# mizeller/OnePose_ST

Hardware: AMD Instinct MI355X
Metric: query frames/sec (2D-3D match+PnP) @ 7k x 4800 d256; 1/2/4/8 GPU (higher is better)
Workload: dtype bf16x3 (split-bf16 MFMA, f32 accumulate)

## Files before the change

### onepose_st_amd/csrc/prep.hip

```cpp
#include "tile.h"

namespace {

__global__ __launch_bounds__(256) void pe_add_transpose_kernel(const float* __restrict__ feat, const float* __restrict__ pe,
                                                               float* __restrict__ out, int Cc, int M) {
    __shared__ float tile[32][33];
    const int tx = threadIdx.x & 31, ty = threadIdx.x >> 5;
    const int m0 = blockIdx.x * 32, c0 = blockIdx.y * 32, b = blockIdx.z;
    const float* f = feat + (size_t)b * Cc * M;
#pragma unroll
    for (int k = 0; k < 4; ++k) {
        const int c = c0 + ty + 8 * k, m = m0 + tx;
        tile[ty + 8 * k][tx] = (c < Cc && m < M) ? f[(size_t)c * M + m] : 0.f;
    }
    __syncthreads();
    float* o = out + (size_t)b * M * Cc;
#pragma unroll
    for (int k = 0; k < 4; ++k) {
        const int m = m0 + ty + 8 * k, c = c0 + tx;
        if (m < M && c < Cc) o[(size_t)m * Cc + c] = tile[tx][ty + 8 * k] + (pe ? pe[(size_t)m * Cc + c] : 0.f);
    }
}

constexpr int KS_THREADS = 1024, KS_WAVES = KS_THREADS / 64;

__global__ __launch_bounds__(KS_THREADS) void kpt_stats_kernel(const float* __restrict__ kpts, long long bs, float* __restrict__ stats, int B, int N) {
    __shared__ float red[KS_WAVES][9];
    const int b = blockIdx.x, tid = threadIdx.x, lane = tid & 63, wave = tid >> 6;
    const float* k = kpts + (size_t)b * bs;
    float s[3] = {0.f, 0.f, 0.f}, mn[3] = {INFINITY, INFINITY, INFINITY}, mx[3] = {-INFINITY, -INFINITY, -INFINITY};
#pragma unroll 4
    for (int i = tid; i < N; i += KS_THREADS) {
#pragma unroll
        for (int d = 0; d < 3; ++d) {
            const float v = k[(size_t)i * 3 + d];
            s[d] += v; mn[d] = fminf(mn[d], v); mx[d] = fmaxf(mx[d], v);
        }
    }
#pragma unroll
    for (int d = 0; d < 3; ++d) {
        s[d] = wave_sum(s[d]);
        mx[d] = wave_max(mx[d]);
        mn[d] = -wave_max(-mn[d]);
    }
    if (lane == 0) {
#pragma unroll
        for (int d = 0; d < 3; ++d) { red[wave][d] = s[d]; red[wave][3 + d] = mn[d]; red[wave][6 + d] = mx[d]; }
    }
    __syncthreads();
    if (tid == 0) {
        float ext = 0.f;
        for (int d = 0; d < 3; ++d) {
            float sum = 0.f, lo = INFINITY, hi = -INFINITY;
            for (int w = 0; w < KS_WAVES; ++w) {
                sum += red[w][d];
                lo = fminf(lo, red[w][3 + d]);
                hi = fmaxf(hi, red[w][6 + d]);
            }
            stats[4 * b + d] = sum / (float)N;
            ext = fmaxf(ext, hi - lo);
        }
        stats[4 * b + 3] = 0.f;
        if (b == 0) stats[4 * B] = ext * 0.6f;
    }
}

constexpr int KD = 256;
constexpr int L0 = 8 + OPHIP_PAD, L1 = 32 + OPHIP_PAD, L2 = 64 + OPHIP_PAD, L3 = 128 + OPHIP_PAD, LO = KD + OPHIP_PAD;

struct KptArgs {
    const float* kpts; long long kbs;
    const float* stats;
    const float* desc; long long dbs;
    const f32x4 *w1, *w2, *w3, *w4;
    const float *b1, *b2, *b3, *b4;
    float* out;
    int B, N;
};

__global__ __launch_bounds__(256) void kpt_encode_kernel(KptArgs p) {
    extern __shared__ __attribute__((aligned(16))) float smem[];
    float* A0 = smem;
    float* A1 = A0 + 32 * L0;
    float* A2 = A1 + 32 * L1;
    float* A3 = A2 + 32 * L2;
    float* Ot = A3 + 32 * L3;
    const int tid = threadIdx.x, lane = tid & 63, wave = tid >> 6;
    const int r = lane & 31, h = lane >> 5;
    const int n0 = blockIdx.x * 32, b = blockIdx.y;
    const float scaling = p.stats[4 * p.B];
    if (tid < 32 * 8) {
        const int row = tid >> 3, d = tid & 7;
        float v = 0.f;
        if (d < 3 && n0 + row < p.N) v = (p.kpts[(size_t)b * p.kbs + (size_t)(n0 + row) * 3 + d] - p.stats[4 * b + d]) / scaling;
        A0[row * L0 + d] = v;
    }
    const float* dsc = p.desc + (size_t)b * p.dbs;
    {
        float dv[KD * 32 / 256];
        const int n = tid & 31, cb = tid >> 5;
        const bool live = n0 + n < p.N;
#pragma unroll
        for (int k = 0; k < KD * 32 / 256; ++k) dv[k] = live ? dsc[(size_t)(cb + 8 * k) * p.N + n0 + n] : 0.f;
#pragma unroll
        for (int k = 0; k < KD * 32 / 256; ++k) Ot[n * LO + cb + 8 * k] = dv[k];
    }
    __syncthreads();
    if (wave == 0) {
        f32x16 acc[1] = {zero16()};
        gemm_lds_x_packed<1, 1>(acc, A0 + r * L0 + 4 * h, 1, p.w1 + lane, 64);
        const float bias = p.b1[r];
#pragma unroll
        for (int reg = 0; reg < 16; ++reg) acc[0][reg] += bias;
        acc_to_lds(acc[0], A1, L1, 0, lane);
    }
    __syncthreads();
    rows_layernorm<32, false, true>(A1, L1, nullptr, nullptr, 1e-5f, wave, lane);
    __syncthreads();
    if (wave < 2) {
        f32x16 acc[1] = {zero16()};
        gemm_lds_x_packed<1>(acc, A1 + r * L1 + 4 * h, 4, p.w2 + (size_t)wave * 4 * 64 + lane, 4 * 64);
        const float bias = p.b2[32 * wave + r];
#pragma unroll
        for (int reg = 0; reg < 16; ++reg) acc[0][reg] += bias;
        acc_to_lds(acc[0], A2, L2, 32 * wave, lane);
    }
    __syncthreads();
    rows_layernorm<64, false, true>(A2, L2, nullptr, nullptr, 1e-5f, wave, lane);
    __syncthreads();
    {
        f32x16 acc[1] = {zero16()};
        gemm_lds_x_packed<1>(acc, A2 + r * L2 + 4 * h, 8, p.w3 + (size_t)wave * 8 * 64 + lane, 8 * 64);
        const float bias = p.b3[32 * wave + r];
#pragma unroll
        for (int reg = 0; reg < 16; ++reg) acc[0][reg] += bias;
        acc_to_lds(acc[0], A3, L3, 32 * wave, lane);
    }
    __syncthreads();
    rows_layernorm<128, false, true>(A3, L3, nullptr, nullptr, 1e-5f, wave, lane);
    __syncthreads();
    {
        f32x16 acc[2] = {zero16(), zero16()};
        gemm_lds_x_packed<2>(acc, A3 + r * L3 + 4 * h, 16, p.w4 + (size_t)(2 * wave) * 16 * 64 + lane, 16 * 64);
#pragma unroll
        for (int t = 0; t < 2; ++t) {
            const int c = 64 * wave + 32 * t + r;
            const float bias = p.b4[c];
#pragma unroll
            for (int reg = 0; reg < 16; ++reg) {
                const int row = acc_row(reg, h);
                Ot[row * LO + c] = Ot[row * LO + c] + (acc[t][reg] + bias);
            }
        }
    }
    __syncthreads();
    float* o = p.out + (size_t)b * p.N * KD;
    for (int rr = 0; rr < 8; ++rr) {
        const int row = 8 * wave + rr;
        if (n0 + row < p.N)
            *reinterpret_cast<f32x4*>(o + (size_t)(n0 + row) * KD + 4 * lane) = *reinterpret_cast<const f32x4*>(Ot + row * LO + 4 * lane);
    }
}

__global__ __launch_bounds__(256) void transpose_cl_kernel(const float* __restrict__ in, float* __restrict__ out, int Cc, int L) {
    __shared__ float tile[32][33];
    const int tx = threadIdx.x & 31, ty = threadIdx.x >> 5;
    const int l0 = blockIdx.x * 32, c0 = blockIdx.y * 32, b = blockIdx.z;
#pragma unroll
    for (int k = 0; k < 4; ++k) {
        const int c = c0 + ty + 8 * k, l = l0 + tx;
        tile[ty + 8 * k][tx] = (c < Cc && l < L) ? in[((size_t)b * Cc + c) * L + l] : 0.f;
    }
    __syncthreads();
#pragma unroll
    for (int k = 0; k < 4; ++k) {
        const int l = l0 + ty + 8 * k, c = c0 + tx;
        if (l < L && c < Cc) out[((size_t)b * L + l) * Cc + c] = tile[tx][ty + 8 * k];
    }
}

__global__ __launch_bounds__(256) void transpose_c128_kernel(const float* __restrict__ in, float* __restrict__ out, int L) {
    __shared__ float tile[128][33];
    const int tid = threadIdx.x, l0 = blockIdx.x * 32, b = blockIdx.y;
    const float* src = in + (size_t)b * 128 * L;
    const int lx = tid & 31, cy = tid >> 5;
#pragma unroll
    for (int k = 0; k < 16; ++k) {
        const int c = cy + 8 * k;
        tile[c][lx] = (l0 + lx < L) ? src[(size_t)c * L + l0 + lx] : 0.f;
    }
    __syncthreads();
    float* dst = out + (size_t)b * L * 128;
    const int p = tid >> 3, q0 = tid & 7;
    if (l0 + p < L) {
#pragma unroll
        for (int m = 0; m < 4; ++m) {
            const int q = q0 + 8 * m;
            f32x4 v = {tile[4 * q][p], tile[4 * q + 1][p], tile[4 * q + 2][p], tile[4 * q + 3][p]};
            *reinterpret_cast<f32x4*>(dst + (size_t)(l0 + p) * 128 + 4 * q) = v;
        }
    }
}

__global__ __launch_bounds__(256) void crop_resize_kernel(const unsigned char* __restrict__ img, int H, int W, int x0, int y0, int wb, int hb,
                                                          int S, float* __restrict__ out) {
    const int X = blockIdx.x * 32 + (threadIdx.x & 31), Y = blockIdx.y * 8 + (threadIdx.x >> 5);
    if (X >= S || Y >= S) return;
    const float inv = (float)wb / (float)S;
    const float u = ((float)X - 0.5f * (float)S) * inv + 0.5f * (float)wb;
    const float v = ((float)Y - 0.5f * (float)S) * inv + 0.5f * (float)hb;
    const float fu = floorf(u), fv = floorf(v);
    const int i0 = (int)fu, j0 = (int)fv;
    const float a = u - fu, b = v - fv;
    auto px = [&](int i, int j) -> float {
        if (i < 0 || i >= wb || j < 0 || j >= hb) return 0.f;
        const int x = x0 + i, y = y0 + j;
        return (x >= 0 && x < W && y >= 0 && y < H) ? (float)img[(size_t)y * W + x] : 0.f;
    };
    const float val = (1.f - b) * ((1.f - a) * px(i0, j0) + a * px(i0 + 1, j0)) + b * ((1.f - a) * px(i0, j0 + 1) + a * px(i0 + 1, j0 + 1));
    out[(size_t)Y * S + X] = fminf(fmaxf(rintf(val), 0.f), 255.f) / 255.0f;
}

}

extern "C" int ophip_crop_resize_gray(const unsigned char* image, int H, int W, int x0, int y0, int x1, int y1, int S, float* out, void* stream) {
    if (!image || !out) return ophip_bad_arg(__func__, "null pointer");
    if (H < 1 || W < 1 || S < 1 || x1 <= x0 || y1 <= y0) return ophip_bad_arg(__func__, "bad sizes (need x1 > x0, y1 > y0)");
    OPHIP_LAUNCH("crop_resize", (hipStream_t)stream, crop_resize_kernel, dim3((S + 31) / 32, (S + 7) / 8), dim3(256), 0, (hipStream_t)stream,
                 image, H, W, x0, y0, x1 - x0, y1 - y0, S, out);
    OPHIP_CHECK_LAUNCH();
    return 0;
}

extern "C" int ophip_pe_add_transpose(const float* feat_nchw, const float* pe_nlc, float* out_nlc, int B, int C, int M, void* stream) {
    if (!feat_nchw || !out_nlc) return ophip_bad_arg(__func__, "null pointer");
    if (B < 1 || C < 1 || M < 1) return ophip_bad_arg(__func__, "bad sizes");
    OPHIP_LAUNCH("pe_add_transpose", (hipStream_t)stream, pe_add_transpose_kernel, dim3((M + 31) / 32, (C + 31) / 32, B), dim3(256), 0, (hipStream_t)stream,
                       feat_nchw, pe_nlc, out_nlc, C, M);
    OPHIP_CHECK_LAUNCH();
    return 0;
}

extern "C" int ophip_transpose_cl(const float* in_bcl, float* out_blc, int B, int C, int L, void* stream) {
    if (!in_bcl || !out_blc) return ophip_bad_arg(__func__, "null pointer");
    if (C == 128) {
        OPHIP_LAUNCH("transpose_cl", (hipStream_t)stream, transpose_c128_kernel, dim3((L + 31) / 32, B), dim3(256), 0, (hipStream_t)stream, in_bcl, out_blc, L);
        OPHIP_CHECK_LAUNCH();
        return 0;
    }
    OPHIP_LAUNCH("transpose_cl", (hipStream_t)stream, transpose_cl_kernel, dim3((L + 31) / 32, (C + 31) / 32, B), dim3(256), 0, (hipStream_t)stream, in_bcl, out_blc, C, L);
    OPHIP_CHECK_LAUNCH();
    return 0;
}

extern "C" int ophip_kpt_encode(const float* keypoints3d, long long kpts_bstride, const float* desc_bcn, long long desc_bstride,
                                const float* wpack, float* stats, float* out_bnc, int B, int N, void* stream_) {
    if (!keypoints3d || !desc_bcn || !wpack || !stats || !out_bnc) return ophip_bad_arg(__func__, "null pointer");
    if (B < 1 || N < 1) return ophip_bad_arg(__func__, "bad sizes");
    hipStream_t stream = (hipStream_t)stream_;
    OPHIP_LAUNCH("kpt_stats", stream, kpt_stats_kernel, dim3(B), dim3(KS_THREADS), 0, stream, keypoints3d, kpts_bstride, stats, B, N);
    OPHIP_CHECK_LAUNCH();
    KptArgs a;
    a.kpts = keypoints3d; a.kbs = kpts_bstride; a.stats = stats; a.desc = desc_bcn; a.dbs = desc_bstride;
    const float* w = wpack;
    a.w1 = reinterpret_cast<const f32x4*>(w); w += 32 * 8;
    a.w2 = reinterpret_cast<const f32x4*>(w); w += 64 * 32;
    a.w3 = reinterpret_cast<const f32x4*>(w); w += 128 * 64;
    a.w4 = reinterpret_cast<const f32x4*>(w); w += 256 * 128;
    a.b1 = w; a.b2 = w + 32; a.b3 = w + 96; a.b4 = w + 224;
    a.out = out_bnc; a.B = B; a.N = N;
    const size_t lds = (size_t)(32 * (L0 + L1 + L2 + L3 + LO)) * sizeof(float);
    if (int rc = ophip_lds_attr(reinterpret_cast<const void*>(kpt_encode_kernel), lds, "hipFuncSetAttribute(kpt_encode)")) return rc;
    OPHIP_LAUNCH("kpt_encode", stream, kpt_encode_kernel, dim3((N + 31) / 32, B), dim3(256), lds, stream, a);
    OPHIP_CHECK_LAUNCH();
    return 0;
}
```

Baseline: 1546.

## Fuse keypoint stats into encoder, vectorize transposes, preload MLP weights into registers

Removes the separate kpt_stats launch: every encoder block now recomputes the keypoint mean and extent itself (redundant per-block reduction over N points) before normalizing. The MLP weights are preloaded into registers, with a ring prefetch for the last layer, and the layernorm+ReLU uses DPP/permlane reductions. The descriptor loads are vectorized. The transpose and pe-add kernels are rewritten to use f32x4 loads and stores with a rotated LDS tile. This cuts one launch and several memory passes, but adds redundant reduction work in each block and more register pressure.

```diff
diff --git a/onepose_st_amd/csrc/prep.hip b/onepose_st_amd/csrc/prep.hip
--- a/onepose_st_amd/csrc/prep.hip
+++ b/onepose_st_amd/csrc/prep.hip
@@ -2,8 +2,72 @@
 
 namespace {
 
+constexpr int TR_C = 128;
+constexpr int TR_T_FINE = 64;
+constexpr int TR_T_PE = 32;
+
+template <int T, bool VEC, bool PE>
+__device__ __forceinline__ void transpose_tile(const float* __restrict__ src, const float* __restrict__ pe, float* __restrict__ dst,
+                                               int C, int L, int l0, int c0, f32x4* tile) {
+    constexpr int LQ = T / 4, CQ = 256 / LQ, PASS = 32 / CQ, ROT = 16 / LQ, ROWS = T / 8;
+    static_assert(T == 32 || T == 64, "tile of 32 or 64 positions");
+    const int tid = threadIdx.x;
+    const int lq = tid % LQ, cq = tid / LQ, l = l0 + 4 * lq;
+    f32x4 v[PASS][4];
+#pragma unroll
+    for (int p = 0; p < PASS; ++p)
+#pragma unroll
+        for (int i = 0; i < 4; ++i) {
+            const float* s = src + (size_t)(c0 + 4 * (cq + CQ * p) + i) * L;
+            if (VEC) {
+                v[p][i] = *reinterpret_cast<const f32x4*>(s + (l < L ? l : 0));
+            } else {
+#pragma unroll
+                for (int j = 0; j < 4; ++j) v[p][i][j] = s[l + j < L ? l + j : 0];
+            }
+        }
+    const int q = tid & 31, r8 = tid >> 5;
+    f32x4 o[ROWS];
+#pragma unroll
+    for (int k = 0; k < ROWS; ++k) o[k] = f32x4{0.f, 0.f, 0.f, 0.f};
+    if (PE && pe) {
+#pragma unroll
+        for (int k = 0; k < ROWS; ++k) {
+            const int lr = l0 + r8 + 8 * k;
+            o[k] = *reinterpret_cast<const f32x4*>(pe + (size_t)(lr < L ? lr : 0) * C + c0 + 4 * q);
+        }
+    }
+#pragma unroll
+    for (int p = 0; p < PASS; ++p)
+#pragma unroll
+        for (int j = 0; j < 4; ++j) {
+            const f32x4 t = {v[p][0][j], v[p][1][j], v[p][2][j], v[p][3][j]};
+            tile[(4 * lq + j) * 32 + ((cq + CQ * p + ROT * lq) & 31)] = t;
+        }
+    __syncthreads();
+#pragma unroll
+    for (int k = 0; k < ROWS; ++k) {
+        const int row = r8 + 8 * k;
+        const f32x4 t = tile[row * 32 + ((q + ROT * (row >> 2)) & 31)];
+        o[k] = PE ? t + o[k] : t;
+    }
+#pragma unroll
+    for (int k = 0; k < ROWS; ++k) {
+        const int lr = l0 + r8 + 8 * k;
+        if (lr < L) *reinterpret_cast<f32x4*>(dst + (size_t)lr * C + c0 + 4 * q) = o[k];
+    }
+}
+
+template <bool VEC>
 __global__ __launch_bounds__(256) void pe_add_transpose_kernel(const float* __restrict__ feat, const float* __restrict__ pe,
                                                                float* __restrict__ out, int Cc, int M) {
+    __shared__ f32x4 tile[TR_T_PE * 32];
+    const int b = blockIdx.z;
+    transpose_tile<TR_T_PE, VEC, true>(feat + (size_t)b * Cc * M, pe, out + (size_t)b * M * Cc, Cc, M, blockIdx.x * TR_T_PE, blockIdx.y * TR_C, tile);
+}
+
+__global__ __launch_bounds__(256) void pe_add_transpose_generic_kernel(const float* __restrict__ feat, const float* __restrict__ pe,
+                                                                       float* __restrict__ out, int Cc, int M) {
     __shared__ float tile[32][33];
     const int tx = threadIdx.x & 31, ty = threadIdx.x >> 5;
     const int m0 = blockIdx.x * 32, c0 = blockIdx.y * 32, b = blockIdx.z;
@@ -23,62 +87,157 @@
 }
 
 constexpr int KS_THREADS = 1024, KS_WAVES = KS_THREADS / 64;
-
-__global__ __launch_bounds__(KS_THREADS) void kpt_stats_kernel(const float* __restrict__ kpts, long long bs, float* __restrict__ stats, int B, int N) {
-    __shared__ float red[KS_WAVES][9];
-    const int b = blockIdx.x, tid = threadIdx.x, lane = tid & 63, wave = tid >> 6;
-    const float* k = kpts + (size_t)b * bs;
-    float s[3] = {0.f, 0.f, 0.f}, mn[3] = {INFINITY, INFINITY, INFINITY}, mx[3] = {-INFINITY, -INFINITY, -INFINITY};
-#pragma unroll 4
-    for (int i = tid; i < N; i += KS_THREADS) {
-#pragma unroll
-        for (int d = 0; d < 3; ++d) {
-            const float v = k[(size_t)i * 3 + d];
-            s[d] += v; mn[d] = fminf(mn[d], v); mx[d] = fmaxf(mx[d], v);
-        }
-    }
-#pragma unroll
-    for (int d = 0; d < 3; ++d) {
-        s[d] = wave_sum(s[d]);
-        mx[d] = wave_max(mx[d]);
-        mn[d] = -wave_max(-mn[d]);
-    }
-    if (lane == 0) {
-#pragma unroll
-        for (int d = 0; d < 3; ++d) { red[wave][d] = s[d]; red[wave][3 + d] = mn[d]; red[wave][6 + d] = mx[d]; }
-    }
-    __syncthreads();
-    if (tid == 0) {
-        float ext = 0.f;
-        for (int d = 0; d < 3; ++d) {
-            float sum = 0.f, lo = INFINITY, hi = -INFINITY;
-            for (int w = 0; w < KS_WAVES; ++w) {
-                sum += red[w][d];
-                lo = fminf(lo, red[w][3 + d]);
-                hi = fmaxf(hi, red[w][6 + d]);
-            }
-            stats[4 * b + d] = sum / (float)N;
-            ext = fmaxf(ext, hi - lo);
-        }
-        stats[4 * b + 3] = 0.f;
-        if (b == 0) stats[4 * B] = ext * 0.6f;
-    }
-}
-
 constexpr int KD = 256;
 constexpr int L0 = 8 + OPHIP_PAD, L1 = 32 + OPHIP_PAD, L2 = 64 + OPHIP_PAD, L3 = 128 + OPHIP_PAD, LO = KD + OPHIP_PAD;
 
 struct KptArgs {
     const float* kpts; long long kbs;
-    const float* stats;
+    float* stats;
     const float* desc; long long dbs;
     const f32x4 *w1, *w2, *w3, *w4;
     const float *b1, *b2, *b3, *b4;
     float* out;
     int B, N;
+    int dvec;
 };
 
-__global__ __launch_bounds__(256) void kpt_encode_kernel(KptArgs p) {
+__device__ __forceinline__ float lane_xor4(float v) {
+    const int u = __builtin_bit_cast(int, v);
+    int t = __builtin_amdgcn_update_dpp(u, u, 0x104, 0xf, 0x5, false);
+    t = __builtin_amdgcn_update_dpp(t, u, 0x114, 0xf, 0xa, false);
+    return __builtin_bit_cast(float, t);
+}
+__device__ __forceinline__ float wave_sum_from16(float v) {
+    const unsigned u = __builtin_bit_cast(unsigned, v);
+    auto a = __builtin_amdgcn_permlane16_swap(u, u, false, false);
+    const unsigned a0 = a[0], a1 = a[1];
+    v = __builtin_bit_cast(float, a0) + __builtin_bit_cast(float, a1);
+    v += dpp_f<0x128>(v);
+    v += lane_xor4(v);
+    v += dpp_f<0x4E>(v);
+    v += dpp_f<0xB1>(v);
+    return v;
+}
+__device__ __forceinline__ float wave_sum_valu(float v) { return wave_sum_from16(swap32_sum(v)); }
+
+__device__ __forceinline__ void kpt_partials(const float* __restrict__ k, int N, float (*red)[9], int wave, int lane) {
+    float s[4][3], mn[4][3], mx[4][3];
+#pragma unroll
+    for (int v = 0; v < 4; ++v)
+#pragma unroll
+        for (int d = 0; d < 3; ++d) { s[v][d] = 0.f; mn[v][d] = INFINITY; mx[v][d] = -INFINITY; }
+#pragma unroll 2
+    for (int i0 = 64 * wave + lane; i0 < N; i0 += KS_THREADS) {
+#pragma unroll
+        for (int v = 0; v < 4; ++v) {
+            const int i = i0 + 256 * v;
+            const bool in = i < N;
+            const float* kp = k + (size_t)(in ? i : 0) * 3;
+#pragma unroll
+            for (int d = 0; d < 3; ++d) {
+                const float x = kp[d];
+                s[v][d] = in ? s[v][d] + x : s[v][d];
+                mn[v][d] = in ? fminf(mn[v][d], x) : mn[v][d];
+                mx[v][d] = in ? fmaxf(mx[v][d], x) : mx[v][d];
+            }
+        }
+    }
+    float lo[4][3], hi[4][3];
+#pragma unroll
+    for (int v = 0; v < 4; ++v)
+#pragma unroll
+        for (int d = 0; d < 3; ++d) {
+            s[v][d] = wave_sum_valu(s[v][d]);
+            hi[v][d] = wave_max_dpp(mx[v][d]);
+            lo[v][d] = -wave_max_dpp(-mn[v][d]);
+        }
+    if (lane == 0) {
+#pragma unroll
+        for (int v = 0; v < 4; ++v)
+#pragma unroll
+            for (int d = 0; d < 3; ++d) { red[wave + 4 * v][d] = s[v][d]; red[wave + 4 * v][3 + d] = lo[v][d]; red[wave + 4 * v][6 + d] = hi[v][d]; }
+    }
+}
+
+template <int KB>
+__device__ __forceinline__ void gemm_lds_x_regs(f32x16& acc, const float* lds_a, const f32x4 (&w)[KB]) {
+#pragma unroll
+    for (int kb = 0; kb < KB; ++kb) acc = mfma4(*reinterpret_cast<const f32x4*>(lds_a + 8 * kb), w[kb], acc);
+}
+
+template <int NT, int PD>
+__device__ __forceinline__ void ring_fill(f32x4 (&ring)[PD][NT], const f32x4* __restrict__ wfrag, int tstride) {
+#pragma unroll
+    for (int p = 0; p < PD; ++p)
+#pragma unroll
+        for (int t = 0; t < NT; ++t) ring[p][t] = wfrag[(size_t)t * tstride + (size_t)p * 64];
+}
+template <int NT, int PD>
+__device__ __forceinline__ void gemm_lds_x_ring(f32x16 (&acc)[NT], const float* lds_a, int kblocks, const f32x4* __restrict__ wfrag, int tstride,
+                                                f32x4 (&ring)[PD][NT]) {
+    for (int kb0 = 0; kb0 < kblocks; kb0 += PD) {
+#pragma unroll
+        for (int p = 0; p < PD; ++p) {
+            const int kb = kb0 + p;
+            const f32x4 a = *reinterpret_cast<const f32x4*>(lds_a + 8 * kb);
+#pragma unroll
+            for (int t = 0; t < NT; ++t) acc[t] = mfma4(a, ring[p][t], acc[t]);
+            const int kn = (kb + PD < kblocks) ? kb + PD : kblocks - 1;
+#pragma unroll
+            for (int t = 0; t < NT; ++t) ring[p][t] = wfrag[(size_t)t * tstride + (size_t)kn * 64];
+            __builtin_amdgcn_sched_barrier(0);
+        }
+    }
+}
+
+template <int C>
+__device__ __forceinline__ float norm_rstd(float qsum, float eps) { return 1.0f / sqrtf(qsum * (1.0f / C) + eps); }
+
+template <int C>
+__device__ __forceinline__ void rows_norm_relu8(float* img, int ld, float eps, int wave, int lane) {
+#pragma clang fp contract(off)
+    constexpr int PER = (C + 63) / 64;
+    static_assert(C % 64 == 0 ? PER <= 2 : PER == 1, "one or two whole elements per lane, or part of a wave");
+    float d[8][PER], s[8], q[8];
+#pragma unroll
+    for (int rr = 0; rr < 8; ++rr) {
+        const float* row = img + (8 * wave + rr) * ld;
+        s[rr] = 0.f;
+#pragma unroll
+        for (int e = 0; e < PER; ++e) {
+            const int c = lane + 64 * e;
+            d[rr][e] = (c < C) ? row[c] : 0.f;
+            s[rr] += d[rr][e];
+        }
+    }
+#pragma unroll
+    for (int rr = 0; rr < 8; ++rr) {
+        const float sum = wave_sum_valu(s[rr]);
+#pragma unroll
+        for (int e = 0; e < PER; ++e) d[rr][e] = __builtin_fmaf(sum, -(1.0f / C), d[rr][e]);
+        const float d0 = (lane < C) ? d[rr][0] : 0.f;
+        if (PER == 1) {
+            q[rr] = wave_sum_from16(__builtin_fmaf(d0, d0, __shfl_xor(d0 * d0, 32, 64)));
+        } else {
+            q[rr] = wave_sum_valu(__builtin_fmaf(d0, d0, d[rr][PER - 1] * d[rr][PER - 1]));
+        }
+    }
+#pragma unroll
+    for (int rr = 0; rr < 8; ++rr) {
+        float* row = img + (8 * wave + rr) * ld;
+        const float rstd = norm_rstd<C>(q[rr], eps);
+#pragma unroll
+        for (int e = 0; e < PER; ++e) {
+            const int c = lane + 64 * e;
+            if (c < C) {
+                const float y = d[rr][e] * rstd;
+                row[c] = (y != y) ? y : fmaxf(y, 0.f);
+            }
+        }
+    }
+}
+
+__global__ __launch_bounds__(256) OPHIP_WAVES_PER_SIMD(2, 2) void kpt_encode_kernel(KptArgs p) {
     extern __shared__ __attribute__((aligned(16))) float smem[];
     float* A0 = smem;
     float* A1 = A0 + 32 * L0;
@@ -88,73 +247,125 @@
     const int tid = threadIdx.x, lane = tid & 63, wave = tid >> 6;
     const int r = lane & 31, h = lane >> 5;
     const int n0 = blockIdx.x * 32, b = blockIdx.y;
-    const float scaling = p.stats[4 * p.B];
-    if (tid < 32 * 8) {
-        const int row = tid >> 3, d = tid & 7;
-        float v = 0.f;
-        if (d < 3 && n0 + row < p.N) v = (p.kpts[(size_t)b * p.kbs + (size_t)(n0 + row) * 3 + d] - p.stats[4 * b + d]) / scaling;
-        A0[row * L0 + d] = v;
-    }
+    float (*red_b)[9] = reinterpret_cast<float (*)[9]>(A3);
+    float (*red_0)[9] = red_b;
+    const float* kp = p.kpts + (size_t)b * p.kbs;
+    kpt_partials(kp, p.N, red_b, wave, lane);
+    if (b != 0 && p.kbs != 0) {
+        red_0 = red_b + KS_WAVES;
+        kpt_partials(p.kpts, p.N, red_0, wave, lane);
+    }
+    const int krow = tid >> 3, kd = tid & 7;
+    const bool klive = kd < 3 && n0 + krow < p.N;
+    const float kv = kp[klive ? (size_t)(n0 + krow) * 3 + kd : 0];
+    f32x4 w1[1], w2[4], w3[8];
+    const int w12 = wave < 2 ? wave : 0;
+    w1[0] = p.w1[lane];
+    const float bias1 = p.b1[r];
+#pragma unroll
+    for (int kb = 0; kb < 4; ++kb) w2[kb] = p.w2[(size_t)w12 * 4 * 64 + kb * 64 + lane];
+    const float bias2 = p.b2[32 * w12 + r];
+#pragma unroll
+    for (int kb = 0; kb < 8; ++kb) w3[kb] = p.w3[(size_t)wave * 8 * 64 + kb * 64 + lane];
+    const float bias3 = p.b3[32 * wave + r];
     const float* dsc = p.desc + (size_t)b * p.dbs;
+    float dv[KD * 32 / 256];
+    if (p.dvec) {
+        const int nq = n0 + 4 * (tid & 7);
+        const float* d0 = dsc + (size_t)(tid >> 3) * p.N + (nq < p.N ? nq : p.N - 4);
+#pragma unroll
+        for (int k = 0; k < 8; ++k) {
+            const f32x4 t = *reinterpret_cast<const f32x4*>(d0 + (size_t)(32 * k) * p.N);
+#pragma unroll
+            for (int j = 0; j < 4; ++j) dv[4 * k + j] = t[j];
+        }
+    } else {
+        const int dn = tid & 31;
+        const float* d0 = dsc + (size_t)(tid >> 5) * p.N + (n0 + dn < p.N ? n0 + dn : p.N - 1);
+#pragma unroll
+        for (int k = 0; k < KD * 32 / 256; ++k) dv[k] = d0[(size_t)(8 * k) * p.N];
+    }
+    const float bias4[2] = {p.b4[64 * wave + r], p.b4[64 * wave + 32 + r]};
+    __syncthreads();
+    float centre[3], ext = 0.f;
+#pragma unroll
+    for (int d = 0; d < 3; ++d) {
+        float sum = 0.f, lo = INFINITY, hi = -INFINITY;
+#pragma unroll
+        for (int w = 0; w < KS_WAVES; ++w) {
+            sum += red_b[w][d];
+            lo = fminf(lo, red_0[w][3 + d]);
+            hi = fmaxf(hi, red_0[w][6 + d]);
+        }
+        centre[d] = sum / (float)p.N;
+        ext = fmaxf(ext, hi - lo);
+    }
+    const float scaling = ext * 0.6f;
+    if (blockIdx.x == 0 && tid == 0) {
+        p.stats[4 * b] = centre[0]; p.stats[4 * b + 1] = centre[1]; p.stats[4 * b + 2] = centre[2]; p.stats[4 * b + 3] = 0.f;
+        if (b == 0) p.stats[4 * p.B] = scaling;
+    }
+    A0[krow * L0 + kd] = klive ? (kv - (kd == 0 ? centre[0] : kd == 1 ? centre[1] : centre[2])) / scaling : 0.f;
+    __syncthreads();
+    if (wave == 0) {
+        f32x16 acc = zero16();
+        gemm_lds_x_regs<1>(acc, A0 + r * L0 + 4 * h, w1);
+#pragma unroll
+        for (int reg = 0; reg < 16; ++reg) acc[reg] += bias1;
+        acc_to_lds(acc, A1, L1, 0, lane);
+    }
+    __syncthreads();
+    rows_norm_relu8<32>(A1, L1, 1e-5f, wave, lane);
+    __syncthreads();
+    if (wave < 2) {
+        f32x16 acc = zero16();
+        gemm_lds_x_regs<4>(acc, A1 + r * L1 + 4 * h, w2);
+#pragma unroll
+        for (int reg = 0; reg < 16; ++reg) acc[reg] += bias2;
+        acc_to_lds(acc, A2, L2, 32 * wave, lane);
+    }
+    __syncthreads();
+    rows_norm_relu8<64>(A2, L2, 1e-5f, wave, lane);
+    __syncthreads();
     {
-        float dv[KD * 32 / 256];
-        const int n = tid & 31, cb = tid >> 5;
-        const bool live = n0 + n < p.N;
-#pragma unroll
-        for (int k = 0; k < KD * 32 / 256; ++k) dv[k] = live ? dsc[(size_t)(cb + 8 * k) * p.N + n0 + n] : 0.f;
-#pragma unroll
-        for (int k = 0; k < KD * 32 / 256; ++k) Ot[n * LO + cb + 8 * k] = dv[k];
-    }
-    __syncthreads();
-    if (wave == 0) {
-        f32x16 acc[1] = {zero16()};
-        gemm_lds_x_packed<1, 1>(acc, A0 + r * L0 + 4 * h, 1, p.w1 + lane, 64);
-        const float bias = p.b1[r];
-#pragma unroll
-        for (int reg = 0; reg < 16; ++reg) acc[0][reg] += bias;
-        acc_to_lds(acc[0], A1, L1, 0, lane);
-    }
-    __syncthreads();
-    rows_layernorm<32, false, true>(A1, L1, nullptr, nullptr, 1e-5f, wave, lane);
-    __syncthreads();
-    if (wave < 2) {
-        f32x16 acc[1] = {zero16()};
-        gemm_lds_x_packed<1>(acc, A1 + r * L1 + 4 * h, 4, p.w2 + (size_t)wave * 4 * 64 + lane, 4 * 64);
-        const float bias = p.b2[32 * wave + r];
-#pragma unroll
-        for (int reg = 0; reg < 16; ++reg) acc[0][reg] += bias;
-        acc_to_lds(acc[0], A2, L2, 32 * wave, lane);
-    }
-    __syncthreads();
-    rows_layernorm<64, false, true>(A2, L2, nullptr, nullptr, 1e-5f, wave, lane);
-    __syncthreads();
-    {
-        f32x16 acc[1] = {zero16()};
-        gemm_lds_x_packed<1>(acc, A2 + r * L2 + 4 * h, 8, p.w3 + (size_t)wave * 8 * 64 + lane, 8 * 64);
-        const float bias = p.b3[32 * wave + r];
-#pragma unroll
-        for (int reg = 0; reg < 16; ++reg) acc[0][reg] += bias;
-        acc_to_lds(acc[0], A3, L3, 32 * wave, lane);
-    }
-    __syncthreads();
-    rows_layernorm<128, false, true>(A3, L3, nullptr, nullptr, 1e-5f, wave, lane);
+        f32x16 acc = zero16();
+        gemm_lds_x_regs<8>(acc, A2 + r * L2 + 4 * h, w3);
+#pragma unroll
+        for (int reg = 0; reg < 16; ++reg) acc[reg] += bias3;
+        acc_to_lds(acc, A3, L3, 32 * wave, lane);
+    }
+    if (p.dvec) {
+#pragma unroll
+        for (int k = 0; k < 8; ++k)
+#pragma unroll
+            for (int j = 0; j < 4; ++j) Ot[(4 * (tid & 7) + j) * LO + (tid >> 3) + 32 * k] = dv[4 * k + j];
+    } else {
+#pragma unroll
+        for (int k = 0; k < KD * 32 / 256; ++k) Ot[(tid & 31) * LO + (tid >> 5) + 8 * k] = dv[k];
+    }
+    constexpr int PD = 4;
+    const f32x4* w4 = p.w4 + (size_t)(2 * wave) * 16 * 64 + lane;
+    f32x4 ring[PD][2];
+    ring_fill<2, PD>(ring, w4, 16 * 64);
+    __syncthreads();
+    rows_norm_relu8<128>(A3, L3, 1e-5f, wave, lane);
     __syncthreads();
     {
         f32x16 acc[2] = {zero16(), zero16()};
-        gemm_lds_x_packed<2>(acc, A3 + r * L3 + 4 * h, 16, p.w4 + (size_t)(2 * wave) * 16 * 64 + lane, 16 * 64);
+        gemm_lds_x_ring<2, PD>(acc, A3 + r * L3 + 4 * h, 16, w4, 16 * 64, ring);
 #pragma unroll
         for (int t = 0; t < 2; ++t) {
             const int c = 64 * wave + 32 * t + r;
-            const float bias = p.b4[c];
 #pragma unroll
             for (int reg = 0; reg < 16; ++reg) {
                 const int row = acc_row(reg, h);
-                Ot[row * LO + c] = Ot[row * LO + c] + (acc[t][reg] + bias);
+                Ot[row * LO + c] = Ot[row * LO + c] + (acc[t][reg] + bias4[t]);
             }
         }
     }
     __syncthreads();
     float* o = p.out + (size_t)b * p.N * KD;
+#pragma unroll
     for (int rr = 0; rr < 8; ++rr) {
         const int row = 8 * wave + rr;
         if (n0 + row < p.N)
@@ -179,28 +390,14 @@
     }
 }
 
+template <bool VEC>
 __global__ __launch_bounds__(256) void transpose_c128_kernel(const float* __restrict__ in, float* __restrict__ out, int L) {
-    __shared__ float tile[128][33];
-    const int tid = threadIdx.x, l0 = blockIdx.x * 32, b = blockIdx.y;
-    const float* src = in + (size_t)b * 128 * L;
-    const int lx = tid & 31, cy = tid >> 5;
-#pragma unroll
-    for (int k = 0; k < 16; ++k) {
-        const int c = cy + 8 * k;
-        tile[c][lx] = (l0 + lx < L) ? src[(size_t)c * L + l0 + lx] : 0.f;
-    }
-    __syncthreads();
-    float* dst = out + (size_t)b * L * 128;
-    const int p = tid >> 3, q0 = tid & 7;
-    if (l0 + p < L) {
-#pragma unroll
-        for (int m = 0; m < 4; ++m) {
-            const int q = q0 + 8 * m;
-            f32x4 v = {tile[4 * q][p], tile[4 * q + 1][p], tile[4 * q + 2][p], tile[4 * q + 3][p]};
-            *reinterpret_cast<f32x4*>(dst + (size_t)(l0 + p) * 128 + 4 * q) = v;
-        }
-    }
-}
+    __shared__ f32x4 tile[TR_T_FINE * 32];
+    const int b = blockIdx.y;
+    transpose_tile<TR_T_FINE, VEC, false>(in + (size_t)b * 128 * L, nullptr, out + (size_t)b * L * 128, 128, L, blockIdx.x * TR_T_FINE, 0, tile);
+}
+
+inline bool aligned16(const void* p) { return (reinterpret_cast<uintptr_t>(p) & 15) == 0; }
 
 __global__ __launch_bounds__(256) void crop_resize_kernel(const unsigned char* __restrict__ img, int H, int W, int x0, int y0, int wb, int hb,
                                                           int S, float* __restrict__ out) {
@@ -235,20 +432,34 @@
 extern "C" int ophip_pe_add_transpose(const float* feat_nchw, const float* pe_nlc, float* out_nlc, int B, int C, int M, void* stream) {
     if (!feat_nchw || !out_nlc) return ophip_bad_arg(__func__, "null pointer");
     if (B < 1 || C < 1 || M < 1) return ophip_bad_arg(__func__, "bad sizes");
-    OPHIP_LAUNCH("pe_add_transpose", (hipStream_t)stream, pe_add_transpose_kernel, dim3((M + 31) / 32, (C + 31) / 32, B), dim3(256), 0, (hipStream_t)stream,
-                       feat_nchw, pe_nlc, out_nlc, C, M);
+    hipStream_t s = (hipStream_t)stream;
+    if (C % TR_C == 0 && aligned16(out_nlc) && aligned16(pe_nlc)) {
+        const dim3 grid((M + TR_T_PE - 1) / TR_T_PE, C / TR_C, B);
+        if (M % 4 == 0 && aligned16(feat_nchw))
+            OPHIP_LAUNCH("pe_add_transpose", s, pe_add_transpose_kernel<true>, grid, dim3(256), 0, s, feat_nchw, pe_nlc, out_nlc, C, M);
+        else
+            OPHIP_LAUNCH("pe_add_transpose", s, pe_add_transpose_kernel<false>, grid, dim3(256), 0, s, feat_nchw, pe_nlc, out_nlc, C, M);
+    } else {
+        OPHIP_LAUNCH("pe_add_transpose", s, pe_add_transpose_generic_kernel, dim3((M + 31) / 32, (C + 31) / 32, B), dim3(256), 0, s,
+                     feat_nchw, pe_nlc, out_nlc, C, M);
+    }
     OPHIP_CHECK_LAUNCH();
     return 0;
 }
 
 extern "C" int ophip_transpose_cl(const float* in_bcl, float* out_blc, int B, int C, int L, void* stream) {
     if (!in_bcl || !out_blc) return ophip_bad_arg(__func__, "null pointer");
-    if (C == 128) {
-        OPHIP_LAUNCH("transpose_cl", (hipStream_t)stream, transpose_c128_kernel, dim3((L + 31) / 32, B), dim3(256), 0, (hipStream_t)stream, in_bcl, out_blc, L);
+    hipStream_t s = (hipStream_t)stream;
+    if (C == 128 && aligned16(out_blc)) {
+        const dim3 grid((L + TR_T_FINE - 1) / TR_T_FINE, B);
+        if (L % 4 == 0 && aligned16(in_bcl))
+            OPHIP_LAUNCH("transpose_cl", s, transpose_c128_kernel<true>, grid, dim3(256), 0, s, in_bcl, out_blc, L);
+        else
+            OPHIP_LAUNCH("transpose_cl", s, transpose_c128_kernel<false>, grid, dim3(256), 0, s, in_bcl, out_blc, L);
         OPHIP_CHECK_LAUNCH();
         return 0;
     }
-    OPHIP_LAUNCH("transpose_cl", (hipStream_t)stream, transpose_cl_kernel, dim3((L + 31) / 32, (C + 31) / 32, B), dim3(256), 0, (hipStream_t)stream, in_bcl, out_blc, C, L);
+    OPHIP_LAUNCH("transpose_cl", s, transpose_cl_kernel, dim3((L + 31) / 32, (C + 31) / 32, B), dim3(256), 0, s, in_bcl, out_blc, C, L);
     OPHIP_CHECK_LAUNCH();
     return 0;
 }
@@ -258,8 +469,6 @@
     if (!keypoints3d || !desc_bcn || !wpack || !stats || !out_bnc) return ophip_bad_arg(__func__, "null pointer");
     if (B < 1 || N < 1) return ophip_bad_arg(__func__, "bad sizes");
     hipStream_t stream = (hipStream_t)stream_;
-    OPHIP_LAUNCH("kpt_stats", stream, kpt_stats_kernel, dim3(B), dim3(KS_THREADS), 0, stream, keypoints3d, kpts_bstride, stats, B, N);
-    OPHIP_CHECK_LAUNCH();
     KptArgs a;
     a.kpts = keypoints3d; a.kbs = kpts_bstride; a.stats = stats; a.desc = desc_bcn; a.dbs = desc_bstride;
     const float* w = wpack;
@@ -269,6 +478,7 @@
     a.w4 = reinterpret_cast<const f32x4*>(w); w += 256 * 128;
     a.b1 = w; a.b2 = w + 32; a.b3 = w + 96; a.b4 = w + 224;
     a.out = out_bnc; a.B = B; a.N = N;
+    a.dvec = N % 4 == 0 && aligned16(desc_bcn) && desc_bstride % 4 == 0;
     const size_t lds = (size_t)(32 * (L0 + L1 + L2 + L3 + LO)) * sizeof(float);
     if (int rc = ophip_lds_attr(reinterpret_cast<const void*>(kpt_encode_kernel), lds, "hipFuncSetAttribute(kpt_encode)")) return rc;
     OPHIP_LAUNCH("kpt_encode", stream, kpt_encode_kernel, dim3((N + 31) / 32, B), dim3(256), lds, stream, a);
```

After: 1537, median of 2. Within noise of the previous version (-0.6%).
